# fengweie/UDA_CLR

Measured on AMD Instinct MI355X. Metric: training images/sec (512x512, src+tgt) at 1/2/4/8 MI355X; val Dice vs ref, higher is better.
Workload: dtype f32

## Files before the change

include/uda_clr_hip.h:

```cpp
#ifndef UDA_CLR_HIP_H
#define UDA_CLR_HIP_H

#include <stdint.h>

#ifdef __cplusplus
extern "C" {
#endif

#define UDA_STAT_SLOTS 16

#define UDA_ACT_NONE 0
#define UDA_ACT_RELU 1
#define UDA_ACT_RELU6 2

typedef struct uda_src {
    const float* x;
    int64_t ldx;
    int32_t N, H, W, C;
    const float* scale;
    const float* shift;
    int32_t act;
    int32_t _pad;
    const uint8_t* mask;
    int64_t ldm;
// ... 104 lines not shown
uint64_t uda_conv3n_workspace_bytes(int Cin, int Cout);
int uda_conv3n_wgrad(const uda_src_t* src, const float* dy, int64_t lddy, int Cout, int stride, float* dw,
                     float* workspace, uint64_t workspace_bytes, void* stream);

int uda_relayout_s2d(const float* w, int O, int C, int dgrad, float* out, void* stream);
int uda_s2d_fwd(const float* src, int64_t ld_src, int nchw_in, int N, int Hs, int Ws, int C, int valid_h,
                int valid_w, float slope, float* z, int64_t ld_z, int Hz, int Wz, void* stream);
int uda_s2d_bwd(const float* dz, const float* z_sign, int64_t ld_z, int Hz, int Wz, float slope, int N, int Hs,
                int Ws, int C, int valid_h, int valid_w, float* dst, int64_t ld_dst, int nchw_out, void* stream);
int uda_s2d_bwd_gate(const float* dz, int64_t ld_z, int Hz, int Wz, const float* gate_rows, int64_t ld_gate, float slope,
                     int N, int Hs, int Ws, int C, int valid_h, int valid_w, float* dst, int64_t ld_dst, void* stream);
int uda_x3_pack_s2d_fwd(const float* src, int64_t ld_src, int N, int Hs, int Ws, int C, int valid_h, int valid_w, float slope,
                        int Hz, int Wz, void* out, void* stream);
int uda_x3_pack_s2d_bwd(const float* dz, int64_t ld_z, int Hz, int Wz, const float* gate_rows, int64_t ld_gate, float slope,
                        int N, int Hs, int Ws, int C, int valid_h, int valid_w, void* out, void* stream);

int uda_bn_finalize(const double* stats, int C, double count, const float* gamma, const float* beta,
                    float* running_mean, float* running_var, float momentum, float eps, float* scale,
                    float* shift, float* mean, float* invstd, void* stream);
int uda_bn_running_replay(const float* mean, const float* invstd, int C, double count, int k, float momentum,
                          float eps, float* running_mean, float* running_var, void* stream);
int uda_bn_eval_coeffs(const float* gamma, const float* beta, const float* running_mean,
                       const float* running_var, int C, float eps, float* scale, float* shift,
                       void* stream);
int uda_tn_gain(const double* stats0, const double* stats1, int C, double count0, double count1, float eps,
                float* scale0, float* shift0, float* scale1, float* shift1, float* gain, void* stream);
int uda_tn_eval_coeffs(const float* gamma, const float* beta, const float* running_mean_source,
                       const float* running_var_source, const float* running_mean_target,
                       const float* running_var_target, int C, float eps, float* scale, float* shift, void* stream);
int uda_bn_apply(const uda_src_t* src, const float* residual, int64_t ldr, float* out, int64_t ldo,
// ... 154 lines not shown
```

uda_clr_amd/acts.py:

```python
from __future__ import annotations

from dataclasses import dataclass, field
from typing import Optional

import torch

from .abi import CONSTANTS

ACT_NONE, ACT_RELU, ACT_RELU6 = (CONSTANTS["UDA_ACT_" + a] for a in ("NONE", "RELU", "RELU6"))


def round4(c: int) -> int:
    return (c + 3) // 4 * 4


@dataclass
class BNRec:
    key: str
    mean: torch.Tensor
    invstd: torch.Tensor
    count: float
    q1_border: bool = False
    gain: Optional[torch.Tensor] = None
    frozen: bool = False
# ... 62 lines not shown
    R, T, Cc = w_rtc.shape
    if round4(Cc) < K_CHUNK:
        out = w_rtc.new_zeros(R, T, round4(Cc))
        out[:, :, :Cc] = w_rtc
        return out
    ncc = (Cc + K_CHUNK - 1) // K_CHUNK
    out = w_rtc.new_zeros(R, T, ncc * K_CHUNK)
    out[:, :, :Cc] = w_rtc
    return out.reshape(R, T, ncc, K_CHUNK).permute(0, 2, 1, 3).reshape(R, ncc * T, K_CHUNK).contiguous()


def conv_weight_shape(rows: int, ksize: int, channels: int):
    if ksize == 1 or round4(channels) < K_CHUNK:
        return (rows, ksize * ksize, round4(channels))
    return (rows, ((channels + K_CHUNK - 1) // K_CHUNK) * ksize * ksize, K_CHUNK)
```

uda_clr_amd/csrc/conv_plan.h:

```cpp
#pragma once
#include <stdlib.h>
#include "igemm_args.h"

enum ConvFamily {
    CF_NONE,
    CF_STREAM,
    CF_COUT1,
    CF_HEADS,
    CF_FEW,
    CF_LOW,
    CF_NARROW,
    CF_WS,
    CF_X3,
    CF_X3_TAIL,
    CF_WGRAD,
    CF_WGRAD_WS,
    CF_WGRAD_X3,
    CF_COUNT
};

struct ConvPlan {
    int family;
    const char* error;
    int bm, bn;
// ... 17 lines not shown
    int red_q;
    int stride, Ho, Wo;
    int64_t P;
    int Kc, Jtot;
    size_t lds;
    uint64_t ws_bytes;
};

constexpr size_t igc_tile_bytes(int bm, int bn) { return (size_t)(bm + bn) * IG_LD * sizeof(float); }
constexpr size_t ws_lds_bytes(int bm, int bn) { return 2 * igc_tile_bytes(bm, bn); }
constexpr size_t x3_lds_bytes(int bm, int bn) { return (size_t)2 * (bm + bn) * X3_ROW * 2; }
constexpr size_t wg_ws_lds_bytes(bool big) { return (size_t)2 * WG_BKP * (big ? 512 : 256) * sizeof(float); }
constexpr size_t wg_x3_lds_bytes(int bm, int bn) { return (size_t)2 * 3 * 16 * ((bm * 2 + 64) + (bn * 2 + 64)); }

int launch_conv_ws(ConvKArgs& k, const ConvPlan& p, hipStream_t st);
int launch_conv_x3(const ConvKArgs& k, const ConvPlan& p, const void* x3_src, const void* x3_w, void* ws, hipStream_t st);
int launch_wgrad_ws(WgradKArgs& k, const WgradPlan& p, hipStream_t st);
int launch_wgrad_x3(const WgradKArgs& k, const WgradPlan& p, const void* x3_src, const void* x3_dy, hipStream_t st);

static inline int uda_k_row(int C, int ksize) {
    const int Kc = ((C + 3) / 4) * 4;
    if (ksize == 1 || Kc < IG_BK) return ksize * ksize * Kc;
    return ((Kc + IG_BK - 1) / IG_BK) * ksize * ksize * IG_BK;
}

static bool plan_stream(const uda_conv_args_t* a, int64_t P, int& kh, int& nb) {
    if (a->ksize != 1 || (a->stride > 1) || a->src.mask || a->bias || P < 32768) return false;
    if (!uda_aligned16(a->src.x) || a->src.ldx % 4 || (a->src.C != 16 && a->src.C != 24 && a->src.C != 32)) return false;
    if (P * a->ldy >= ((int64_t)1 << 29) || (a->addend && P * a->ld_add >= ((int64_t)1 << 29))) return false;
    const int C = a->src.C, Cout = a->Cout;
    kh = C / 2;
// ... 218 lines not shown
```

uda_clr_amd/csrc/igemm_args.h:

```cpp
#pragma once
#include "common.h"

struct ConvKArgs {
    uda_src_t src;
    const float* w;
    int Cout, ksize, dil, Kc, Ktot;
    int cen;
    const float* bias;
    const float* addend;
    int64_t ld_add;
    float* y;
    int64_t ldy;
    double* stats;
    int nMt, nNt;
    int debug;
    int x3;
    int stride, Ho, Wo;
};

struct WgradKArgs {
    uda_src_t src;
    const float* dy;
    int64_t lddy;
    int Cout, ksize, dil, Kc, Jtot;
    int cen;
    float* slab;
    int nCot, nJt, chunks_per_split, nchunks;
    int x3;
    int stride, Ho, Wo;
};

#define IG_BK 32
#define IG_LD 36
#define WG_BKP 32
// ... 4 lines not shown
```

uda_clr_amd/csrc/igemm_conv.hip:

```cpp
#include <algorithm>
#include "common.h"
#include "conv_plan.h"

typedef float f32x16 __attribute__((ext_vector_type(16)));


#define IGC_MIN_WAVES(TM, TN, PIPE) ((PIPE) ? 2 : ((TM) * (TN) <= 3 ? 4 : 3))
template <int TM, int TN, int WM, int WN, bool PIPE = false, int XF = -1>
__global__ __launch_bounds__(256) void igemm_conv_kernel(ConvKArgs a) {
    constexpr int BM = 32 * TM * WM, BN = 32 * TN * WN;
    constexpr int A_IT = BM / 32, B_IT = BN / 32;
    constexpr int TILE = (BM + BN) * IG_LD;
    extern __shared__ __attribute__((aligned(16))) float smem[];

    const int tid = threadIdx.x, lane = tid & 63, wave = tid >> 6;
    const int wm = wave / WN, wn = wave % WN;
    const int lid = uda_xcd_remap(blockIdx.x, a.nMt * a.nNt);
    const int mt = lid / a.nNt, nt = lid % a.nNt;
    const int H = a.src.H, W = a.src.W, C = a.src.C;
    const int64_t P = (int64_t)a.src.N * H * W;
    const int64_t m0 = (int64_t)mt * BM;
    const int n0 = nt * BN;

    const int lrow = tid >> 3, kv = (tid & 7) * 4;
// ... 584 lines not shown
        case 122: return launch_stream<12, 2>(k, p.P, st);
        case 123: return launch_stream<12, 3>(k, p.P, st);
        case 125: return launch_stream<12, 5>(k, p.P, st);
        default: return launch_stream<16, 3>(k, p.P, st);
    }
}

extern "C" int uda_conv_uses_x3(const uda_conv_args_t* a) {
    if (!conv_plannable(a)) return 0;
    const int f = conv_plan(a).family;
    return f == CF_X3 || f == CF_X3_TAIL;
}

extern "C" uint64_t uda_conv_fwd_workspace_bytes(const uda_conv_args_t* a) { return conv_plannable(a) ? conv_plan(a).ws_bytes : 0; }

extern "C" int uda_conv_fwd(const uda_conv_args_t* a, void* stream) {
    hipStream_t st = (hipStream_t)stream;
    UDA_REQUIRE(a != nullptr, "uda_conv_fwd: null args");
    if (int e = check_src(a->src, "uda_conv_fwd")) return e;
    UDA_REQUIRE(a->ksize >= 1 && a->ksize <= 3, "uda_conv_fwd: ksize must be 1, 2 or 3");
    UDA_REQUIRE(a->ksize != 2 || a->origin == 0 || a->origin == 1, "uda_conv_fwd: origin must be 0 or 1 for ksize 2");
    UDA_REQUIRE(a->Cout > 0 && a->dil >= 1 && a->y && a->w, "uda_conv_fwd: bad args");
    UDA_REQUIRE(uda_aligned16(a->w), "uda_conv_fwd: weights must be 16-byte aligned");
    UDA_REQUIRE(a->ldy >= a->Cout, "uda_conv_fwd: ldy < Cout");
    UDA_REQUIRE(a->stride <= 2, "uda_conv_fwd: stride must be 1 or 2");
    const int64_t Pin = (int64_t)a->src.N * a->src.H * a->src.W;
    UDA_REQUIRE((Pin + 128) * a->src.ldx < ((int64_t)1 << 29) && (Pin + 128) * (a->src.mask ? a->src.ldm : 1) < ((int64_t)1 << 31),
                "uda_conv_fwd: operand too large for 32-bit byte offsets (P * ld must stay below 2^29 elements)");
    const ConvPlan p = conv_plan(a);
    if (p.error) return uda_set_error("%s", p.error);
    ConvKArgs k;
    k.src = a->src;
    k.stride = p.stride; k.Ho = p.Ho; k.Wo = p.Wo;
    k.w = a->w;
    k.Cout = a->Cout;
    k.ksize = a->ksize;
    k.dil = a->dil;
    k.cen = a->ksize == 3 ? 1 : (a->ksize == 2 ? a->origin : 0);
    k.Kc = p.Kc;
    k.Ktot = p.Ktot;
    k.bias = a->bias;
    k.addend = a->addend;
    k.ld_add = a->ld_add;
    k.y = a->y;
    k.ldy = a->ldy;
// ... 1 lines not shown
    k.debug = 0;
    k.x3 = a->mfma == UDA_MFMA_BF16X3;
    switch (p.family) {
        case CF_STREAM: return launch_stream_shape(k, p, st);
        case CF_COUT1:
            hipLaunchKernelGGL(conv_cout1_kernel, dim3(p.grid), dim3(256), 0, st, k);
            UDA_LAUNCH_CHECK("conv_cout1");
            return 0;
        case CF_HEADS:
            if (p.bn == 1) hipLaunchKernelGGL(conv_heads_kernel<1>, dim3(p.grid), dim3(256), p.lds, st, k);
            else hipLaunchKernelGGL(conv_heads_kernel<2>, dim3(p.grid), dim3(256), p.lds, st, k);
            UDA_LAUNCH_CHECK("conv_heads");
            return 0;
        case CF_FEW: case CF_LOW: case CF_NARROW: return launch_conv_tile(k, p, st);
        case CF_WS: return launch_conv_ws(k, p, st);
        case CF_X3: case CF_X3_TAIL: return launch_conv_x3(k, p, a->x3_src, a->x3_w, a->workspace, st);
        default: return uda_set_error("uda_conv_fwd: no kernel planned");
    }
}



template <int TM, int TN, int WM, int WN>
__global__ __launch_bounds__(256) void igemm_wgrad_kernel(WgradKArgs a) {
    constexpr int BM = 32 * TM * WM, BN = 32 * TN * WN;
    constexpr int AV = BM / 4, BV = BN / 4;
    constexpr int ARPP = 256 / AV, BRPP = 256 / BV;
    constexpr int APASS = WGN_BKP / ARPP, BPASS = WGN_BKP / BRPP;
    __shared__ __attribute__((aligned(16))) float smem[WGN_BKP * (BM + BN)];
    float* As = smem;
    float* Bs = smem + WGN_BKP * BM;

    const int tid = threadIdx.x, lane = tid & 63, wave = tid >> 6;
// ... 366 lines not shown
```

uda_clr_amd/csrc/igemm_x3.hip:

```cpp
#include "common.h"
#include "conv_plan.h"

typedef float f32x16 __attribute__((ext_vector_type(16)));
typedef __bf16 bf16x8 __attribute__((ext_vector_type(8)));
typedef __bf16 bf16x2 __attribute__((ext_vector_type(2)));



__device__ __forceinline__ void x3_split2(float v0, float v1, uint32_t& p1, uint32_t& p2, uint32_t& p3) {
    bf16x2 a = {(__bf16)v0, (__bf16)v1};
    p1 = __builtin_bit_cast(uint32_t, a);
    const float r0 = v0 - __builtin_bit_cast(float, p1 << 16), r1 = v1 - __builtin_bit_cast(float, p1 & 0xffff0000u);
    bf16x2 b = {(__bf16)r0, (__bf16)r1};
    p2 = __builtin_bit_cast(uint32_t, b);
    const float s0 = r0 - __builtin_bit_cast(float, p2 << 16), s1 = r1 - __builtin_bit_cast(float, p2 & 0xffff0000u);
    bf16x2 c = {(__bf16)s0, (__bf16)s1};
    p3 = __builtin_bit_cast(uint32_t, c);
}

struct X3PackArgs {
    uda_src_t src;
    int64_t P;
    int nb;
    uint32_t* out;
// ... 119 lines not shown
    const uint32_t* xa;
    const uint32_t* xw;
    int N, H, W, nbA;
    int stride, Ho, Wo;
    int Cout, ksize, dil, cen, nchunks;
    const float* bias;
    const float* addend;
    int64_t ld_add;
    float* y;
    int64_t ldy;
    double* stats;
    int nMt, nNt;
    int debug;
    int tile_off, ksplit, ntiles_main;
    float* partial;
};

template <int KS, int TN, int BM, bool TAIL = false>
__global__ __launch_bounds__(768) void igemm_conv_x3_kernel(X3KArgs a) {
    constexpr int MW = 8, BN = 64 * TN, TM = 2;
    constexpr int WMM = BM / 64, WNN = MW / WMM, TNW = 2 * TN / WNN;
    static_assert(WMM * WNN == MW && (2 * TN) % WNN == 0, "math-wave grid must tile the workgroup tile");
    constexpr int NTHR = (MW + 4) * 64;
    constexpr int A_U = BM * 6 / 256, B_UNITS = BN * 6, B_U = (B_UNITS + 255) / 256;
    static_assert((BM * 6) % 256 == 0, "A units must divide over the 256 loader threads");
    constexpr bool B_FULL = B_UNITS % 256 == 0;
    constexpr int TILE = (BM + BN) * X3_ROW;
    extern __shared__ __attribute__((aligned(16))) __bf16 smem16[];

    const int tid = threadIdx.x, lane = tid & 63, wave = tid >> 6;
    const bool loader = __builtin_amdgcn_readfirstlane(wave) >= MW;
    const int lid = TAIL ? a.tile_off + (int)blockIdx.x / a.ksplit : uda_xcd_remap(blockIdx.x, a.ntiles_main);
    const int mt = lid / a.nNt, nt = lid % a.nNt;
// ... 163 lines not shown
                a.partial + (int64_t)blockIdx.x * (BM * BN), 0, BM * BN * 4, 0x00020000);
            const int pv = ((wm * 64 + 4 * (lane >> 5)) * BN + wn * (32 * TNW) + (lane & 31)) * 4;
#pragma unroll
            for (int j = 0; j < TNW; ++j)
#pragma unroll
                for (int i = 0; i < TM; ++i)
#pragma unroll
                    for (int r = 0; r < 16; ++r) {
                        const float v = acc[i][j][r];
                        __builtin_amdgcn_raw_buffer_store_b32(__builtin_bit_cast(unsigned, v), pres, pv + 128 * j,
                                                              (32 * i + (r & 3) + 8 * (r >> 2)) * (BN * 4), 0);
                    }
            return;
        }
        if constexpr (TAIL) return;
        float s1[TNW], s2[TNW];
#pragma unroll
        for (int j = 0; j < TNW; ++j) s1[j] = s2[j] = 0.f;
        const int rows_left = (int)min((int64_t)BM, P - m0);
        const int ldy4 = (int)a.ldy * 4, lda4 = (int)a.ld_add * 4;
        const __amdgpu_buffer_rsrc_t yres = __builtin_amdgcn_make_buffer_rsrc(
            a.y + m0 * a.ldy, 0, ((rows_left - 1) * (int)a.ldy + a.Cout) * 4, 0x00020000);
        const __amdgpu_buffer_rsrc_t adres = __builtin_amdgcn_make_buffer_rsrc(
            const_cast<float*>(a.addend ? a.addend + m0 * a.ld_add : a.y), 0, a.addend ? ((rows_left - 1) * (int)a.ld_add + a.Cout) * 4 : 0, 0x00020000);
        const int colb = n0 + wn * (32 * TNW) + (lane & 31);
        const int rbase = wm * 64 + 4 * (lane >> 5);
#pragma unroll
        for (int j = 0; j < TNW; ++j) {
            const int col = colb + 32 * j;
            const bool cok = col < a.Cout;
// ... 40 lines not shown
                atomicAdd(&dst[qd * a.Cout + n0 + cl], (double)t);
            }
        }
    }
}

struct X3TailArgs {
    const float* partial;
    int ksplit, tile_off, ntail, nNt, BM, BN, Cout;
    int64_t P;
    const float* bias;
    const float* addend;
    int64_t ld_add;
    float* y;
    int64_t ldy;
};

__global__ __launch_bounds__(256) void x3_tail_reduce_kernel(X3TailArgs a) {
    const int bn4 = a.BN >> 2, per_tile = a.BM * bn4;
    const int64_t total = (int64_t)a.ntail * per_tile;
    for (int64_t e = (int64_t)blockIdx.x * 256 + threadIdx.x; e < total; e += (int64_t)gridDim.x * 256) {
        const int tl = (int)(e / per_tile), q = (int)(e - (int64_t)tl * per_tile), r = q / bn4, c4 = (q - r * bn4) * 4;
        const int lid = a.tile_off + tl, mt = lid / a.nNt, nt = lid - mt * a.nNt;
        const int64_t row = (int64_t)mt * a.BM + r;
        const int col = nt * a.BN + c4;
        if (row >= a.P || col >= a.Cout) continue;
        float4 acc = make_float4(0.f, 0.f, 0.f, 0.f);
        for (int s = 0; s < a.ksplit; ++s) {
            const float4 v = uda_ld4(a.partial + (((int64_t)tl * a.ksplit + s) * a.BM + r) * a.BN + c4);
            acc.x += v.x; acc.y += v.y; acc.z += v.z; acc.w += v.w;
        }
        const float o[4] = {acc.x, acc.y, acc.z, acc.w};
#pragma unroll
        for (int jj = 0; jj < 4; ++jj)
            if (col + jj < a.Cout) {
                float v = o[jj] + (a.bias ? a.bias[col + jj] : 0.f);
                if (a.addend) v += a.addend[row * a.ld_add + col + jj];
                a.y[row * a.ldy + col + jj] = v;
            }
    }
}

template <int KS, int TN, int BM>
static int launch_x3(X3KArgs& k, const ConvPlan& p, float* ws, hipStream_t st) {
    constexpr int BN = 64 * TN;
    static_assert(x3_lds_bytes(BM, BN) <= 160 * 1024, "tile does not fit the 160 KiB LDS");
    k.nMt = uda_cdiv(p.P, BM);
    k.nNt = uda_cdiv(k.Cout, BN);
    k.debug = 0;
#ifdef UDA_DIAG
    static const int dbg = getenv("UDA_X3_DEBUG") ? atoi(getenv("UDA_X3_DEBUG")) : 0;
    k.debug = dbg;
#endif
    k.tile_off = 0; k.ksplit = 1; k.partial = nullptr;
    k.ntiles_main = p.grid;
    if (k.ntiles_main > 0) {
        if (int e = uda_reserve_lds<igemm_conv_x3_kernel<KS, TN, BM>>(p.lds, "igemm_conv_x3")) return e;
        hipLaunchKernelGGL((igemm_conv_x3_kernel<KS, TN, BM>), dim3(k.ntiles_main), dim3(768), p.lds, st, k);
        UDA_LAUNCH_CHECK("igemm_conv_x3");
    }
    if (p.ksplit > 1) {
        k.tile_off = (int)p.full; k.ksplit = p.ksplit; k.partial = ws;
        if (int e = uda_reserve_lds<igemm_conv_x3_kernel<KS, TN, BM, true>>(p.lds, "igemm_conv_x3 (tail)")) return e;
        hipLaunchKernelGGL((igemm_conv_x3_kernel<KS, TN, BM, true>), dim3((int)p.tail * p.ksplit), dim3(768), p.lds, st, k);
        UDA_LAUNCH_CHECK("igemm_conv_x3 (tail)");
        X3TailArgs r;
        r.partial = k.partial; r.ksplit = p.ksplit; r.tile_off = (int)p.full; r.ntail = (int)p.tail; r.nNt = k.nNt; r.BM = BM; r.BN = BN;
        r.Cout = k.Cout; r.P = p.P; r.bias = k.bias; r.addend = k.addend; r.ld_add = k.ld_add; r.y = k.y; r.ldy = k.ldy;
        const int64_t work = (int64_t)p.tail * BM * (BN / 4);
        hipLaunchKernelGGL(x3_tail_reduce_kernel, dim3((int)uda_cdiv(work, 256)), dim3(256), 0, st, r);
        UDA_LAUNCH_CHECK("x3_tail_reduce");
    }
    return 0;
}

static inline int x3_nb(int C) { return uda_cdiv(C, X3_BK); }

extern "C" uint64_t uda_x3_packed_bytes(int64_t rows, int K) { return (uint64_t)rows * x3_nb(K) * 96 + 64; }

extern "C" int uda_x3_pack(const uda_src_t* src, void* out, void* stream) {
    UDA_REQUIRE(src && src->x && out && uda_aligned16(out) && uda_aligned16(src->x) && src->ldx % 4 == 0 && src->C > 0,
                "uda_x3_pack: bad args (16-byte aligned rows)");
    hipStream_t st = (hipStream_t)stream;
// ... 39 lines not shown
    pa.Hs = Hs; pa.Ws = Ws; pa.Cs = C; pa.vh = valid_h; pa.vw = valid_w; pa.Hz = Hz; pa.Wz = Wz; pa.slope = slope;
    const int64_t tot = pa.P * pa.nb * 2;
    const int grid = (int)(uda_cdiv(tot, 256) > 65536 ? 65536 : uda_cdiv(tot, 256));
    hipLaunchKernelGGL(x3_pack_kernel<4>, dim3(grid), dim3(256), 0, (hipStream_t)stream, pa);
    UDA_LAUNCH_CHECK("x3_pack_s2d_bwd");
    return 0;
}

template <int KS>
static int launch_x3_tile(X3KArgs& x, const ConvPlan& p, float* ws, hipStream_t st) {
    if (p.bn == 64) return launch_x3<3, 1, 256>(x, p, ws, st);
    if (p.bm == 256) return p.bn == 256 ? launch_x3<KS, 4, 256>(x, p, ws, st) : launch_x3<KS, 2, 256>(x, p, ws, st);
    return p.bn == 256 ? launch_x3<KS, 4, 128>(x, p, ws, st) : launch_x3<KS, 2, 128>(x, p, ws, st);
}

int launch_conv_x3(const ConvKArgs& k, const ConvPlan& p, const void* x3_src, const void* x3_w, void* ws, hipStream_t st) {
    const int64_t lim = (int64_t)1 << 31;
    const int nbA = x3_nb(k.src.C), nch = uda_cdiv(k.Ktot, X3_BK);
    UDA_REQUIRE(x3_src && x3_w && uda_aligned16(x3_src) && uda_aligned16(x3_w),
                "uda_conv_fwd (bf16x3): the packed operands x3_src / x3_w are missing (uda_x3_pack; uda_conv_uses_x3 tells when they are needed)");
    const int64_t Pin = (int64_t)k.src.N * k.src.H * k.src.W;
    UDA_REQUIRE((Pin + 256) * nbA * 6 < lim / 16 && (int64_t)(k.Cout + 320) * nch * 6 < lim / 16,
                "uda_conv_fwd (bf16x3): operand too large for the 32-bit offsets of the wide-tile kernel");
    X3KArgs x;
    x.xa = reinterpret_cast<const uint32_t*>(x3_src); x.xw = reinterpret_cast<const uint32_t*>(x3_w);
    x.N = k.src.N; x.H = k.src.H; x.W = k.src.W; x.nbA = nbA;
    x.stride = k.stride; x.Ho = k.Ho; x.Wo = k.Wo;
    x.Cout = k.Cout; x.ksize = k.ksize; x.dil = k.dil; x.cen = k.cen; x.nchunks = nch;
    x.bias = k.bias; x.addend = k.addend; x.ld_add = k.ld_add; x.y = k.y; x.ldy = k.ldy; x.stats = k.stats;
    return p.ks == 3 ? launch_x3_tile<3>(x, p, reinterpret_cast<float*>(ws), st) : launch_x3_tile<1>(x, p, reinterpret_cast<float*>(ws), st);
}

typedef short s16x4 __attribute__((ext_vector_type(4)));
typedef short s16x8 __attribute__((ext_vector_type(8)));

struct X3WgArgs {
    const uint32_t* xdy;
    const uint32_t* xs;
    int N, H, W, nbCo, nbC;
    int stride, Ho, Wo;
    int Cout, Jtot, Kc, ksize, dil, cen;
    float* slab;
    int nCot, nJt, cps, nchunks;
};
// ... 209 lines not shown
```

uda_clr_amd/gan_engine.py:

```python
from __future__ import annotations

import torch

from .acts import Act, round4

SLOPE = 0.2


def _zgrid(v):
    return (v + 5) // 2


class PatchDiscriminatorEngine:
    def __init__(self, kernels):
        self.K = kernels

    def forward(self, x, weights, need_grad, pre_op=0, w_share=None):
        K = self.K
        N, Cc, H, W = x.shape
        src, nchw, Hs, Ws, vh, vw, slope = x, True, H, W, H, W, 1.0
        layers = []
        for li, w in enumerate(weights):
            O = w.shape[0]
            if w_share is None:
# ... 16 lines not shown
            else:
                z = torch.empty((N * Hz * Wz, 4 * Cc), dtype=torch.float32, device=x.device)
                if li == 0 and pre_op:
                    K.adv_s2d_fwd(src, pre_op, z)
                else:
                    K.s2d_fwd(src, nchw, N, Hs, Ws, Cc, vh, vw, slope, z)
            y = torch.empty((N * Hz * Wz, round4(O)), dtype=torch.float32, device=x.device)[:, :O]
            K.conv(Act(z, N, Hz, Wz), wf, 2, 1, y, origin=0)
            keep_gate = need_grad and li > 0 and (packed or getattr(K, "mfma", None) == getattr(K, "MFMA_BF16X3", -1))
            layers.append((z if need_grad else None, Cc, Hs, Ws, vh, vw, Hz, Wz, nchw, wd, src if keep_gate else None))
            src, nchw, Hs, Ws, Cc, slope = y, False, Hz, Wz, O, SLOPE
            vh, vw = vh // 2 + 1, vw // 2 + 1
        out = src.reshape(N, Hs, Ws, Cc)[:, :vh, :vw].permute(0, 3, 1, 2)
        return out, ((layers, N, tuple(x.shape), (x if pre_op else None), pre_op) if need_grad else None)

    def backward(self, ctx, gout, weights, need_x, need_w):
        K = self.K
        layers, N, xshape, x_logits, pre_op = ctx
        z5, C5, Hs5, Ws5, vh5, vw5, Hz, Wz, _, _, _ = layers[-1]
        O = weights[-1].shape[0]
        vh, vw = vh5 // 2 + 1, vw5 // 2 + 1
        dy = torch.zeros((N, Hz, Wz, round4(O)), dtype=torch.float32, device=gout.device)
        dy[:, :vh, :vw, :O] = gout.permute(0, 2, 3, 1)
        dy = dy.reshape(N * Hz * Wz, round4(O))[:, :O]
        dws = [None] * len(weights)
        dx = None
        for l in range(len(weights) - 1, -1, -1):
            z, Cc, Hs, Ws, vh, vw, Hz, Wz, nchw, wd, gate = layers[l]
            w = weights[l]
            O = w.shape[0]
            if need_w:
                dwz = torch.empty((O, 4 * Cc, 2, 2), dtype=torch.float32, device=z.device)
                K.conv_wgrad(Act(z, N, Hz, Wz), dy, 2, 1, dwz, origin=0)
                dws[l] = dwz.reshape(O, 2, 2, Cc, 2, 2).permute(0, 3, 4, 1, 5, 2).reshape(O, Cc, 4, 4)
            if l == 0 and not need_x:
                break
            dz = torch.empty_like(z)
            K.conv(Act(dy, N, Hz, Wz), wd, 2, 1, dz, origin=1)
            if nchw:
                dx = torch.empty(xshape, dtype=torch.float32, device=dz.device)
                if pre_op:
                    K.adv_s2d_bwd(dz, x_logits, pre_op, dx)
                else:
                    K.s2d_bwd(dz, None, 1.0, N, Hs, Ws, Cc, vh, vw, dx, True)
            else:
                below = layers[l - 1]
                need_dx_below = (l - 1 > 0) or need_x
                pack_dy = (gate is not None and hasattr(K, "s2d_pack_bwd") and Cc % 8 == 0
                           and (not need_w or K.wgrad_route_x3(N, Hs, Ws, 4 * below[1], Cc, 2))
                           and (not need_dx_below or K.conv_route_x3(N, Hs, Ws, Cc, 4 * below[1], 2)))
                if pack_dy:
                    dy = K.s2d_pack_bwd(dz, gate, SLOPE, N, Hs, Ws, Cc, vh, vw)
                else:
                    dyn = torch.empty((N * Hs * Ws, round4(Cc)), dtype=torch.float32, device=dz.device)[:, :Cc]
                    if gate is not None:
                        K.s2d_bwd(dz, None, SLOPE, N, Hs, Ws, Cc, vh, vw, dyn, False, gate=gate)
                    else:
                        K.s2d_bwd(dz, z, SLOPE, N, Hs, Ws, Cc, vh, vw, dyn, False)
                    dy = dyn
            del dz
        return dx, (dws if need_w else None)
```

uda_clr_amd/kernels.py:

```python
from __future__ import annotations

import ctypes as C
import math
import os
from typing import Optional

import torch

from .abi import CONSTANTS, STRUCTS, SYMBOLS
from .acts import conv_weight_shape, Act, round4

_LIB_PATH = os.path.join(os.path.dirname(os.path.abspath(__file__)), "lib", "libuda_clr_hip.so")
_lib = None

STAT_SLOTS = CONSTANTS["UDA_STAT_SLOTS"]
FDA_MAX_BAND = CONSTANTS["UDA_FDA_MAX_BAND"]
UdaSrc, UdaConvArgs, UdaWgradArgs = STRUCTS["uda_src_t"], STRUCTS["uda_conv_args_t"], STRUCTS["uda_wgrad_args_t"]


def load_library(path: Optional[str] = None):
    global _lib
    if _lib is not None and path is None:
        return _lib
    path = path or _LIB_PATH
    if not os.path.exists(path):
# ... 195 lines not shown
        if x3_channels:
            lim_rows = min(lim_rows, (self.ELEM_LIMIT // 4) // (((x3_channels + 15) // 16) * 6) - 256)
        if N * rows_per_image <= lim_rows:
            return None
        g = lim_rows // rows_per_image
        if g < 1:
            raise UdaError("one image (%d pixels x %d floats per row) exceeds the 32-bit offsets of the conv kernels" % (rows_per_image, widest_ld))
        return [(n0, min(N, n0 + g)) for n0 in range(0, N, g)]

    @staticmethod
    def _act_rows(a: Act, n0, n1):
        ppi = a.P // a.N
        r = slice(n0 * ppi, n1 * ppi)
        return Act(a.x[r], n1 - n0, a.H, a.W, a.scale, a.shift, a.act, None if a.mask is None else a.mask[r], a.mask_scale, a.bn, a.meta)

    def conv(self, src: Act, w, ksize, dil, out, bias=None, addend=None, stats=None, origin=0, stride=1):
        groups = self._image_groups(src.N, src.P // src.N, max(src.x.stride(0), out.stride(0), 0 if addend is None else addend.stride(0),
                                                               0 if src.mask is None else src.mask.stride(0) // 4),
                                    src.C if self.mfma != self.MFMA_F32 else 0)
        Po = src.N * ((src.H - 1) // stride + 1) * ((src.W - 1) // stride + 1)
        if groups is not None:
            ppo = Po // src.N
            for n0, n1 in groups:
                r = slice(n0 * ppo, n1 * ppo)
                self.conv(self._act_rows(src, n0, n1), w, ksize, dil, out[r], bias, None if addend is None else addend[r], stats, origin, stride)
            return
        a = self._conv_args_of(src, w, ksize, dil, out, bias, addend, stats, origin, stride)
        if self.mfma != self.MFMA_F32 and self.lib.uda_conv_uses_x3(C.byref(a)):
            xs = self._packed(src, a.src, out.device)
            xw = getattr(w, "_x3", None)
            if xw is None:
                xw = self.x3_pack_rows(w)
                w._x3 = xw
            a.x3_src, a.x3_w = xs.data_ptr(), xw.data_ptr()
            nws = int(self.lib.uda_conv_fwd_workspace_bytes(C.byref(a)))
            if nws:
                ws = self._ws(out, nws)
                a.workspace, a.workspace_bytes = ws.data_ptr(), nws
            return self._conv_x3(a)
        self._ck(self.lib.uda_conv_fwd(C.byref(a), self._stream()))

    def conv_args(self, usrc: UdaSrc, Cout, ksize, dil=1, origin=0, stride=1, w=None, bias=None, addend=None, ld_add=0, y=None, ldy=0,
                  stats=None) -> UdaConvArgs:
        a = UdaConvArgs()
        a.src, a.origin = usrc, origin
        a.w, a.Cout, a.ksize, a.dil, a.stride = w, Cout, ksize, dil, stride
        a.bias, a.addend, a.ld_add = bias, addend, ld_add
        a.y, a.ldy, a.stats = y, ldy, stats
        a.mfma = self.mfma
        return a

    def _conv_args_of(self, src: Act, w, ksize, dil, out, bias, addend, stats, origin, stride) -> UdaConvArgs:
        Cout = out.shape[1]
        assert w.is_contiguous() and tuple(w.shape) == conv_weight_shape(Cout, ksize, src.C), \
            "weight layout %s does not match conv %dx%d %d->%d" % (tuple(w.shape), ksize, ksize, src.C, Cout)
        assert out.shape[0] == src.N * ((src.H - 1) // stride + 1) * ((src.W - 1) // stride + 1) and stride in (1, 2)
# ... 8 lines not shown
    def route(self, a) -> str:
        buf = C.create_string_buffer(96)
        if isinstance(a, UdaWgradArgs):
            self.lib.uda_conv_wgrad_route(C.byref(a), buf, len(buf))
        else:
            nws = int(self.lib.uda_conv_fwd_workspace_bytes(C.byref(a)))
            if nws and not a.workspace:
                a.workspace, a.workspace_bytes = 16, nws
            self.lib.uda_conv_route(C.byref(a), buf, len(buf))
        return buf.value.decode()

    def conv_route(self, src: Act, w, ksize, dil, out, bias=None, addend=None, stats=None, origin=0, stride=1) -> str:
        return self.route(self._conv_args_of(src, w, ksize, dil, out, bias, addend, stats, origin, stride))

    def _conv_x3(self, a):
        self._ck(self.lib.uda_conv_fwd(C.byref(a), self._stream()))

    def x3_pack(self, usrc: UdaSrc, rows, K, device):
        out = torch.empty(int(self.lib.uda_x3_packed_bytes(rows, K)), dtype=torch.uint8, device=device)
        self._ck(self.lib.uda_x3_pack(C.byref(usrc), out.data_ptr(), self._stream()))
        return out

    def _packed(self, src: Act, usrc: UdaSrc, device):
        xs = getattr(src, "_x3", None)
        raw = not src.lazy
        if xs is None and raw:
            xs = getattr(src.x, "_x3", None)
        if xs is not None and xs.numel() != int(self.lib.uda_x3_packed_bytes(src.P, src.C)):
            raise RuntimeError("bf16x3 packed operand of %d bytes attached to a [%d, %d] matrix (expected %d): stale attachment"
                               % (xs.numel(), src.P, src.C, int(self.lib.uda_x3_packed_bytes(src.P, src.C))))
# ... 1018 lines not shown
```

Baseline: 376.5.

## Fuse space-to-depth backward and LeakyReLU gating into bf16x3 conv epilogue

```diff
diff --git a/include/uda_clr_hip.h b/include/uda_clr_hip.h
--- a/include/uda_clr_hip.h
+++ b/include/uda_clr_hip.h
@@ -142,6 +142,8 @@
                         int Hz, int Wz, void* out, void* stream);
 int uda_x3_pack_s2d_bwd(const float* dz, int64_t ld_z, int Hz, int Wz, const float* gate_rows, int64_t ld_gate, float slope,
                         int N, int Hs, int Ws, int C, int valid_h, int valid_w, void* out, void* stream);
+int uda_conv_fwd_routed(const uda_conv_args_t* a, const float* gate_rows, int64_t ld_gate, float slope, int Hs, int Ws, int C,
+                        int valid_h, int valid_w, float* dst, int64_t ld_dst, void* dst_packed, void* stream);
 
 int uda_bn_finalize(const double* stats, int C, double count, const float* gamma, const float* beta,
                     float* running_mean, float* running_var, float momentum, float eps, float* scale,
diff --git a/uda_clr_amd/acts.py b/uda_clr_amd/acts.py
--- a/uda_clr_amd/acts.py
+++ b/uda_clr_amd/acts.py
@@ -100,3 +100,10 @@
     if ksize == 1 or round4(channels) < K_CHUNK:
         return (rows, ksize * ksize, round4(channels))
     return (rows, ((channels + K_CHUNK - 1) // K_CHUNK) * ksize * ksize, K_CHUNK)
+
+
+class RoutedOut:
+
+    def __init__(self, gate, slope, N, Hs, Ws, C, vh, vw, dst=None, use_workspace=True):
+        self.gate, self.slope, self.N, self.Hs, self.Ws, self.C, self.vh, self.vw = gate, slope, N, Hs, Ws, C, vh, vw
+        self.dst, self.use_workspace = dst, use_workspace
diff --git a/uda_clr_amd/csrc/conv_plan.h b/uda_clr_amd/csrc/conv_plan.h
--- a/uda_clr_amd/csrc/conv_plan.h
+++ b/uda_clr_amd/csrc/conv_plan.h
@@ -55,7 +55,8 @@
 constexpr size_t wg_x3_lds_bytes(int bm, int bn) { return (size_t)2 * 3 * 16 * ((bm * 2 + 64) + (bn * 2 + 64)); }
 
 int launch_conv_ws(ConvKArgs& k, const ConvPlan& p, hipStream_t st);
-int launch_conv_x3(const ConvKArgs& k, const ConvPlan& p, const void* x3_src, const void* x3_w, void* ws, hipStream_t st);
+int launch_conv_x3(const ConvKArgs& k, const ConvPlan& p, const void* x3_src, const void* x3_w, void* ws, const ConvRouteOut* rt,
+                   hipStream_t st);
 int launch_wgrad_ws(WgradKArgs& k, const WgradPlan& p, hipStream_t st);
 int launch_wgrad_x3(const WgradKArgs& k, const WgradPlan& p, const void* x3_src, const void* x3_dy, hipStream_t st);
 
diff --git a/uda_clr_amd/csrc/igemm_args.h b/uda_clr_amd/csrc/igemm_args.h
--- a/uda_clr_amd/csrc/igemm_args.h
+++ b/uda_clr_amd/csrc/igemm_args.h
@@ -18,6 +18,15 @@
     int stride, Ho, Wo;
 };
 
+struct ConvRouteOut {
+    const float* gate;
+    float* dst;
+    uint32_t* packed;
+    int ldg, ldd, nb;
+    int Hs, Ws, C, vh, vw;
+    float slope;
+};
+
 struct WgradKArgs {
     uda_src_t src;
     const float* dy;
diff --git a/uda_clr_amd/csrc/igemm_conv.hip b/uda_clr_amd/csrc/igemm_conv.hip
--- a/uda_clr_amd/csrc/igemm_conv.hip
+++ b/uda_clr_amd/csrc/igemm_conv.hip
@@ -622,13 +622,12 @@
 
 extern "C" uint64_t uda_conv_fwd_workspace_bytes(const uda_conv_args_t* a) { return conv_plannable(a) ? conv_plan(a).ws_bytes : 0; }
 
-extern "C" int uda_conv_fwd(const uda_conv_args_t* a, void* stream) {
-    hipStream_t st = (hipStream_t)stream;
+static int conv_fwd(const uda_conv_args_t* a, const ConvRouteOut* rt, hipStream_t st) {
     UDA_REQUIRE(a != nullptr, "uda_conv_fwd: null args");
     if (int e = check_src(a->src, "uda_conv_fwd")) return e;
     UDA_REQUIRE(a->ksize >= 1 && a->ksize <= 3, "uda_conv_fwd: ksize must be 1, 2 or 3");
     UDA_REQUIRE(a->ksize != 2 || a->origin == 0 || a->origin == 1, "uda_conv_fwd: origin must be 0 or 1 for ksize 2");
-    UDA_REQUIRE(a->Cout > 0 && a->dil >= 1 && a->y && a->w, "uda_conv_fwd: bad args");
+    UDA_REQUIRE(a->Cout > 0 && a->dil >= 1 && (a->y || rt) && a->w, "uda_conv_fwd: bad args");
     UDA_REQUIRE(uda_aligned16(a->w), "uda_conv_fwd: weights must be 16-byte aligned");
     UDA_REQUIRE(a->ldy >= a->Cout, "uda_conv_fwd: ldy < Cout");
     UDA_REQUIRE(a->stride <= 2, "uda_conv_fwd: stride must be 1 or 2");
@@ -637,6 +636,15 @@
                 "uda_conv_fwd: operand too large for 32-bit byte offsets (P * ld must stay below 2^29 elements)");
     const ConvPlan p = conv_plan(a);
     if (p.error) return uda_set_error("%s", p.error);
+    if (rt) {
+        UDA_REQUIRE(p.family == CF_X3 || p.family == CF_X3_TAIL,
+                    "uda_conv_fwd_routed: these arguments do not run on the bf16x3 wide-tile kernel (uda_conv_uses_x3)");
+        UDA_REQUIRE(rt->Hs <= 2 * p.Ho - 2 && rt->Ws <= 2 * p.Wo - 2,
+                    "uda_conv_fwd_routed: source rows beyond 2*Hz - 3 or columns beyond 2*Wz - 3 are reached by no z element and would stay undefined");
+        const int64_t reach = (int64_t)a->src.N * rt->Hs * rt->Ws + 4 * rt->Ws;
+        UDA_REQUIRE(reach * rt->ldg < ((int64_t)1 << 29) && reach * (rt->packed ? (int64_t)rt->nb * 24 : (int64_t)rt->ldd) < ((int64_t)1 << 29),
+                    "uda_conv_fwd_routed: destination too large for 32-bit byte offsets");
+    }
     ConvKArgs k;
     k.src = a->src;
     k.stride = p.stride; k.Ho = p.Ho; k.Wo = p.Wo;
@@ -668,9 +676,33 @@
             return 0;
         case CF_FEW: case CF_LOW: case CF_NARROW: return launch_conv_tile(k, p, st);
         case CF_WS: return launch_conv_ws(k, p, st);
-        case CF_X3: case CF_X3_TAIL: return launch_conv_x3(k, p, a->x3_src, a->x3_w, a->workspace, st);
+        case CF_X3: case CF_X3_TAIL: return launch_conv_x3(k, p, a->x3_src, a->x3_w, a->workspace, rt, st);
         default: return uda_set_error("uda_conv_fwd: no kernel planned");
     }
+}
+
+extern "C" int uda_conv_fwd(const uda_conv_args_t* a, void* stream) { return conv_fwd(a, nullptr, (hipStream_t)stream); }
+
+extern "C" int uda_conv_fwd_routed(const uda_conv_args_t* a, const float* gate_rows, int64_t ld_gate, float slope, int Hs, int Ws, int C,
+                                   int valid_h, int valid_w, float* dst, int64_t ld_dst, void* dst_packed, void* stream) {
+    UDA_REQUIRE(a != nullptr, "uda_conv_fwd_routed: null args");
+    UDA_REQUIRE(a->ksize == 2 && a->origin == 1 && a->stride <= 1, "uda_conv_fwd_routed: needs ksize 2, origin 1, stride 1 (an input gradient on the z grid)");
+    UDA_REQUIRE(!a->stats && !a->bias && !a->addend, "uda_conv_fwd_routed: stats, bias and addend cannot be combined with a routed output");
+    UDA_REQUIRE(C > 0 && C % 32 == 0 && a->Cout == 4 * C,
+                "uda_conv_fwd_routed: needs Cout == 4*C and C %% 32 == 0 (a 32-column block lies inside one (a, b) group, whole 16-wide packed blocks)");
+    UDA_REQUIRE((dst != nullptr) != (dst_packed != nullptr), "uda_conv_fwd_routed: exactly one of dst and dst_packed");
+    UDA_REQUIRE(gate_rows && uda_aligned16(gate_rows) && ld_gate >= C && ld_gate % 4 == 0,
+                "uda_conv_fwd_routed: gate_rows must be 16-byte aligned rows of at least C floats");
+    UDA_REQUIRE(dst ? (uda_aligned16(dst) && ld_dst >= C && ld_dst % 4 == 0) : uda_aligned16(dst_packed),
+                "uda_conv_fwd_routed: dst must be 16-byte aligned (rows of at least C floats)");
+    UDA_REQUIRE(a->src.N > 0 && Hs > 0 && Ws > 0 && valid_h > 0 && valid_w > 0 && valid_h <= Hs && valid_w <= Ws &&
+                a->src.H == (valid_h + 5) / 2 && a->src.W == (valid_w + 5) / 2,
+                "uda_conv_fwd_routed: bad geometry (src must live on the z grid of the valid region)");
+    ConvRouteOut rt;
+    rt.gate = gate_rows; rt.dst = dst; rt.ldg = (int)ld_gate; rt.ldd = (int)ld_dst;
+    rt.packed = reinterpret_cast<uint32_t*>(dst_packed); rt.nb = C / X3_BK;
+    rt.Hs = Hs; rt.Ws = Ws; rt.C = C; rt.vh = valid_h; rt.vw = valid_w; rt.slope = slope;
+    return conv_fwd(a, &rt, (hipStream_t)stream);
 }
 
 
diff --git a/uda_clr_amd/csrc/igemm_x3.hip b/uda_clr_amd/csrc/igemm_x3.hip
--- a/uda_clr_amd/csrc/igemm_x3.hip
+++ b/uda_clr_amd/csrc/igemm_x3.hip
@@ -4,6 +4,7 @@
 typedef float f32x16 __attribute__((ext_vector_type(16)));
 typedef __bf16 bf16x8 __attribute__((ext_vector_type(8)));
 typedef __bf16 bf16x2 __attribute__((ext_vector_type(2)));
+typedef unsigned u32x4 __attribute__((ext_vector_type(4)));
 
 
 
@@ -157,9 +158,19 @@
     int debug;
     int tile_off, ksplit, ntiles_main;
     float* partial;
+    ConvRouteOut rt;
 };
 
-template <int KS, int TN, int BM, bool TAIL = false>
+__device__ __forceinline__ void x3_route_row(int64_t p, int64_t P, int Hz, int Wz, int Hs, int Ws, int& pix, int& h0, int& w0) {
+    pix = 0; h0 = w0 = -(1 << 20);
+    if (p < P) {
+        const int q = (int)p, j = q % Wz, t = q / Wz, i = t % Hz, n = t / Hz;
+        h0 = 2 * i - 2; w0 = 2 * j - 2;
+        pix = (n * Hs + h0) * Ws + w0;
+    }
+}
+
+template <int KS, int TN, int BM, bool TAIL = false, int RT = 0>
 __global__ __launch_bounds__(768) void igemm_conv_x3_kernel(X3KArgs a) {
     constexpr int MW = 8, BN = 64 * TN, TM = 2;
     constexpr int WMM = BM / 64, WNN = MW / WMM, TNW = 2 * TN / WNN;
@@ -353,6 +364,115 @@
             return;
         }
         if constexpr (TAIL) return;
+        if constexpr (RT != 0) {
+            const ConvRouteOut& rt = a.rt;
+            const int wv = __builtin_amdgcn_readfirstlane(wave);
+            int2* tab = reinterpret_cast<int2*>(smem16) + wv * 64;
+            const int dpix = RT == 2 ? rt.nb * 96 : rt.ldd * 4, gpix = rt.ldg * 4;
+            {
+                int pix, h0, w0;
+                x3_route_row(m0 + wm * 64 + lane, P, a.Ho, a.Wo, rt.Hs, rt.Ws, pix, h0, w0);
+                int inb = 0, okb = 0;
+#pragma unroll
+                for (int ab = 0; ab < 4; ++ab) {
+                    const int h = h0 + (ab >> 1), w = w0 + (ab & 1);
+                    const bool in = h >= 0 && h < rt.Hs && w >= 0 && w < rt.Ws;
+                    inb |= (in ? 1 : 0) << ab;
+                    okb |= (in && h < rt.vh && w < rt.vw ? 1 : 0) << ab;
+                }
+                tab[lane] = make_int2(pix * dpix | inb, pix * gpix | okb);
+            }
+            const int64_t npix = (int64_t)a.N * rt.Hs * rt.Ws;
+            const __amdgpu_buffer_rsrc_t dres = RT == 2
+                ? __builtin_amdgcn_make_buffer_rsrc(rt.packed, 0, (int)(npix * dpix), 0x00020000)
+                : __builtin_amdgcn_make_buffer_rsrc(rt.dst, 0, (int)(((npix - 1) * rt.ldd + rt.C) * 4), 0x00020000);
+            const __amdgpu_buffer_rsrc_t gres = __builtin_amdgcn_make_buffer_rsrc(
+                const_cast<float*>(rt.gate), 0, (int)(((npix - 1) * rt.ldg + rt.C) * 4), 0x00020000);
+            const int2* trow = tab + 4 * (lane >> 5);
+            uint32_t* stage = reinterpret_cast<uint32_t*>(smem16) + MW * 64 * 2 + wv * (32 * 48);
+            static_assert(RT != 2 || MW * 64 * 8 + MW * 32 * 192 <= 2 * TILE * 2, "row table and stage must fit the tile images");
+            constexpr int NU = TNW * TM * 2;
+            constexpr bool PARK = RT == 2 && BM == 256 && TN == 4;
+            float* park = reinterpret_cast<float*>(smem16) + MW * 64 * 2 + MW * 32 * 48 + wv * 64 + lane;
+            static_assert(!PARK || MW * 64 * 8 + MW * 32 * 192 + 16 * MW * 64 * 4 <= 2 * TILE * 2, "parked block must fit the tile images");
+            if constexpr (PARK) {
+#pragma unroll
+                for (int r = 0; r < 16; ++r) park[r * (MW * 64)] = acc[TM - 1][TNW - 1][r];
+            }
+            int inbit = 0, okbit = 0, dcol = 0, gcol = 0;
+            auto columns = [&](int u) {
+                const int col0 = __builtin_amdgcn_readfirstlane(n0 + wn * (32 * TNW) + 32 * (u / (2 * TM)));
+                const int ab = (col0 >= rt.C) + (col0 >= 2 * rt.C) + (col0 >= 3 * rt.C) + (col0 >= 4 * rt.C);
+                const int c0 = col0 - ab * rt.C, pixo = (ab >> 1) * rt.Ws + (ab & 1);
+                inbit = okbit = ab < 4 ? 1 << ab : 0;
+                gcol = pixo * gpix + (c0 + (lane & 31)) * 4;
+                dcol = RT == 2 ? pixo * dpix + (c0 >> 4) * 96 : pixo * dpix + (c0 + (lane & 31)) * 4;
+            };
+            auto rl_of = [](int u, int k) { const int r = 8 * (u & 1) + k; return 32 * ((u >> 1) % TM) + (r & 3) + 8 * (r >> 2); };
+            auto issue = [&](int u, float (&g)[8]) {
+                columns(u);
+#pragma unroll
+                for (int k = 0; k < 8; ++k) {
+                    const int2 t = trow[rl_of(u, k)];
+                    g[k] = __builtin_bit_cast(float, __builtin_amdgcn_raw_buffer_load_b32(gres, (t.y & okbit) ? (t.y & ~15) + gcol : OOB, 0, 0));
+                }
+            };
+            auto value = [&](int u, int k, float g, const int2& t) {
+                const int i = (u >> 1) % TM, j = u / (2 * TM), r = 8 * (u & 1) + k;
+                float v = (PARK && i == TM - 1 && j == TNW - 1 ? park[r * (MW * 64)] : acc[i][j][r]) + 0.f;
+                if (!(g > 0.f)) v *= rt.slope;
+                return (t.y & okbit) ? v : 0.f;
+            };
+            auto finish = [&](int u, const float (&g)[8]) {
+                columns(u);
+                if constexpr (RT == 1) {
+#pragma unroll
+                    for (int k = 0; k < 8; ++k) {
+                        const int2 t = trow[rl_of(u, k)];
+                        const float v = value(u, k, g[k], t);
+                        __builtin_amdgcn_raw_buffer_store_b32(__builtin_bit_cast(unsigned, v), dres, (t.x & inbit) ? (t.x & ~15) + dcol : OOB, 0, 0);
+                    }
+                } else {
+                    const bool even = !(lane & 1);
+#pragma unroll
+                    for (int k = 0; k < 8; k += 2) {
+                        if (BM == 256 && k) asm volatile("" ::: "memory");
+                        const int rlA = rl_of(u, k), rlB = rl_of(u, k + 1);
+                        const float vA = value(u, k, g[k], trow[rlA]), vB = value(u, k + 1, g[k + 1], trow[rlB]);
+                        const float mine = even ? vA : vB, other = __shfl_xor(even ? vB : vA, 1);
+                        uint32_t p1, p2, p3;
+                        x3_split2(even ? mine : other, even ? other : mine, p1, p2, p3);
+                        const int rb = ((even ? rlA : rlB) & 31) + 4 * (lane >> 5);
+                        uint32_t* d = stage + rb * 48 + ((lane & 31) >> 4) * 24 + ((lane & 15) >> 1);
+                        d[0] = p1; d[8] = p2; d[16] = p3;
+                    }
+                    if (u & 1) {
+                        const int rband = 32 * ((u >> 1) % TM);
+#pragma unroll
+                        for (int k = 0; k < 6; ++k) {
+                            if (k == 2 || k == 4) asm volatile("" ::: "memory");
+                            const int e = lane + 64 * k, run = e / 12, part = e - run * 12;
+                            const int2 t = tab[rband + run];
+                            const u32x4 v = *reinterpret_cast<const u32x4*>(stage + 4 * e);
+                            __builtin_amdgcn_raw_buffer_store_b128(v, dres, (t.x & inbit) ? (t.x & ~15) + dcol + part * 16 : OOB, 0, 0);
+                        }
+                    }
+                }
+            };
+            constexpr int D = (BM == 256 && TN == 4) ? 2 : 4;
+            float g[D][8];
+#pragma unroll
+            for (int u = 0; u < D - 1; ++u)
+                if (u < NU) issue(u, g[u]);
+#pragma unroll
+            for (int u = 0; u < NU; ++u) {
+                asm volatile("" ::: "memory");
+                if (u + D - 1 < NU) issue(u + D - 1, g[(u + D - 1) % D]);
+                asm volatile("" ::: "memory");
+                finish(u, g[u % D]);
+            }
+            return;
+        }
         float s1[TNW], s2[TNW];
 #pragma unroll
         for (int j = 0; j < TNW; ++j) s1[j] = s2[j] = 0.f;
@@ -423,6 +543,8 @@
     int64_t ld_add;
     float* y;
     int64_t ldy;
+    int routed, Hz, Wz;
+    ConvRouteOut rt;
 };
 
 __global__ __launch_bounds__(256) void x3_tail_reduce_kernel(X3TailArgs a) {
@@ -440,6 +562,34 @@
             acc.x += v.x; acc.y += v.y; acc.z += v.z; acc.w += v.w;
         }
         const float o[4] = {acc.x, acc.y, acc.z, acc.w};
+        if (a.routed) {
+            int pix, h0, w0;
+            x3_route_row(row, a.P, a.Hz, a.Wz, a.rt.Hs, a.rt.Ws, pix, h0, w0);
+            const int ab = col / a.rt.C, c = col - ab * a.rt.C, h = h0 + (ab >> 1), w = w0 + (ab & 1);
+            if (h < 0 || h >= a.rt.Hs || w < 0 || w >= a.rt.Ws) continue;
+            const int64_t px = pix + (ab >> 1) * a.rt.Ws + (ab & 1);
+            float4 v = make_float4(0.f, 0.f, 0.f, 0.f);
+            if (h < a.rt.vh && w < a.rt.vw) {
+                const float4 g = uda_ld4(a.rt.gate + px * a.rt.ldg + c);
+                v = make_float4(o[0] + 0.f, o[1] + 0.f, o[2] + 0.f, o[3] + 0.f);
+                if (!(g.x > 0.f)) v.x *= a.rt.slope;
+                if (!(g.y > 0.f)) v.y *= a.rt.slope;
+                if (!(g.z > 0.f)) v.z *= a.rt.slope;
+                if (!(g.w > 0.f)) v.w *= a.rt.slope;
+            }
+            if (a.rt.packed) {
+                uint32_t p1[2], p2[2], p3[2];
+                x3_split2(v.x, v.y, p1[0], p2[0], p3[0]);
+                x3_split2(v.z, v.w, p1[1], p2[1], p3[1]);
+                uint32_t* d = a.rt.packed + ((px * a.rt.nb + (c >> 4)) * 24 + ((c & 15) >> 1));
+                *reinterpret_cast<uint2*>(d) = make_uint2(p1[0], p1[1]);
+                *reinterpret_cast<uint2*>(d + 8) = make_uint2(p2[0], p2[1]);
+                *reinterpret_cast<uint2*>(d + 16) = make_uint2(p3[0], p3[1]);
+            } else {
+                uda_st4(a.rt.dst + px * a.rt.ldd + c, v);
+            }
+            continue;
+        }
 #pragma unroll
         for (int jj = 0; jj < 4; ++jj)
             if (col + jj < a.Cout) {
@@ -450,7 +600,7 @@
     }
 }
 
-template <int KS, int TN, int BM>
+template <int KS, int TN, int BM, int RT = 0>
 static int launch_x3(X3KArgs& k, const ConvPlan& p, float* ws, hipStream_t st) {
     constexpr int BN = 64 * TN;
     static_assert(x3_lds_bytes(BM, BN) <= 160 * 1024, "tile does not fit the 160 KiB LDS");
@@ -464,8 +614,8 @@
     k.tile_off = 0; k.ksplit = 1; k.partial = nullptr;
     k.ntiles_main = p.grid;
     if (k.ntiles_main > 0) {
-        if (int e = uda_reserve_lds<igemm_conv_x3_kernel<KS, TN, BM>>(p.lds, "igemm_conv_x3")) return e;
-        hipLaunchKernelGGL((igemm_conv_x3_kernel<KS, TN, BM>), dim3(k.ntiles_main), dim3(768), p.lds, st, k);
+        if (int e = uda_reserve_lds<igemm_conv_x3_kernel<KS, TN, BM, false, RT>>(p.lds, "igemm_conv_x3")) return e;
+        hipLaunchKernelGGL((igemm_conv_x3_kernel<KS, TN, BM, false, RT>), dim3(k.ntiles_main), dim3(768), p.lds, st, k);
         UDA_LAUNCH_CHECK("igemm_conv_x3");
     }
     if (p.ksplit > 1) {
@@ -476,6 +626,7 @@
         X3TailArgs r;
         r.partial = k.partial; r.ksplit = p.ksplit; r.tile_off = (int)p.full; r.ntail = (int)p.tail; r.nNt = k.nNt; r.BM = BM; r.BN = BN;
         r.Cout = k.Cout; r.P = p.P; r.bias = k.bias; r.addend = k.addend; r.ld_add = k.ld_add; r.y = k.y; r.ldy = k.ldy;
+        r.routed = RT != 0; r.Hz = k.Ho; r.Wz = k.Wo; r.rt = k.rt;
         const int64_t work = (int64_t)p.tail * BM * (BN / 4);
         hipLaunchKernelGGL(x3_tail_reduce_kernel, dim3((int)uda_cdiv(work, 256)), dim3(256), 0, st, r);
         UDA_LAUNCH_CHECK("x3_tail_reduce");
@@ -545,7 +696,14 @@
     return p.bn == 256 ? launch_x3<KS, 4, 128>(x, p, ws, st) : launch_x3<KS, 2, 128>(x, p, ws, st);
 }
 
-int launch_conv_x3(const ConvKArgs& k, const ConvPlan& p, const void* x3_src, const void* x3_w, void* ws, hipStream_t st) {
+template <int RT>
+static int launch_x3_routed(X3KArgs& x, const ConvPlan& p, float* ws, hipStream_t st) {
+    if (p.bm == 256) return p.bn == 256 ? launch_x3<3, 4, 256, RT>(x, p, ws, st) : launch_x3<3, 2, 256, RT>(x, p, ws, st);
+    return p.bn == 256 ? launch_x3<3, 4, 128, RT>(x, p, ws, st) : launch_x3<3, 2, 128, RT>(x, p, ws, st);
+}
+
+int launch_conv_x3(const ConvKArgs& k, const ConvPlan& p, const void* x3_src, const void* x3_w, void* ws, const ConvRouteOut* rt,
+                   hipStream_t st) {
     const int64_t lim = (int64_t)1 << 31;
     const int nbA = x3_nb(k.src.C), nch = uda_cdiv(k.Ktot, X3_BK);
     UDA_REQUIRE(x3_src && x3_w && uda_aligned16(x3_src) && uda_aligned16(x3_w),
@@ -559,6 +717,11 @@
     x.stride = k.stride; x.Ho = k.Ho; x.Wo = k.Wo;
     x.Cout = k.Cout; x.ksize = k.ksize; x.dil = k.dil; x.cen = k.cen; x.nchunks = nch;
     x.bias = k.bias; x.addend = k.addend; x.ld_add = k.ld_add; x.y = k.y; x.ldy = k.ldy; x.stats = k.stats;
+    x.rt = rt ? *rt : ConvRouteOut{};
+    if (rt) {
+        UDA_REQUIRE(p.ks == 3 && p.bn >= 128, "uda_conv_fwd_routed: no routed epilogue for this tile");
+        return rt->packed ? launch_x3_routed<2>(x, p, reinterpret_cast<float*>(ws), st) : launch_x3_routed<1>(x, p, reinterpret_cast<float*>(ws), st);
+    }
     return p.ks == 3 ? launch_x3_tile<3>(x, p, reinterpret_cast<float*>(ws), st) : launch_x3_tile<1>(x, p, reinterpret_cast<float*>(ws), st);
 }
 
diff --git a/uda_clr_amd/gan_engine.py b/uda_clr_amd/gan_engine.py
--- a/uda_clr_amd/gan_engine.py
+++ b/uda_clr_amd/gan_engine.py
@@ -2,7 +2,7 @@
 
 import torch
 
-from .acts import Act, round4
+from .acts import Act, RoutedOut, round4
 
 SLOPE = 0.2
 
@@ -54,7 +54,7 @@
         out = src.reshape(N, Hs, Ws, Cc)[:, :vh, :vw].permute(0, 3, 1, 2)
         return out, ((layers, N, tuple(x.shape), (x if pre_op else None), pre_op) if need_grad else None)
 
-    def backward(self, ctx, gout, weights, need_x, need_w):
+    def backward(self, ctx, gout, weights, need_x, need_w, fuse_route=True):
         K = self.K
         layers, N, xshape, x_logits, pre_op = ctx
         z5, C5, Hs5, Ws5, vh5, vw5, Hz, Wz, _, _, _ = layers[-1]
@@ -75,6 +75,17 @@
                 dws[l] = dwz.reshape(O, 2, 2, Cc, 2, 2).permute(0, 3, 4, 1, 5, 2).reshape(O, Cc, 4, 4)
             if l == 0 and not need_x:
                 break
+            below = None if nchw else layers[l - 1]
+            pack_dy = (not nchw and gate is not None and hasattr(K, "s2d_pack_bwd") and Cc % 8 == 0
+                       and (not need_w or K.wgrad_route_x3(N, Hs, Ws, 4 * below[1], Cc, 2))
+                       and (not ((l - 1 > 0) or need_x) or K.conv_route_x3(N, Hs, Ws, Cc, 4 * below[1], 2)))
+            if (fuse_route and not nchw and gate is not None and Cc % 32 == 0 and hasattr(K, "conv_routed")
+                    and (pack_dy or l == 1) and K.conv_route_x3(N, Hz, Wz, O, 4 * Cc, 2)):
+                dst = None if pack_dy else torch.empty((N * Hs * Ws, round4(Cc)), dtype=torch.float32, device=gout.device)[:, :Cc]
+                shape = torch.empty((N * Hz * Wz, 4 * Cc), dtype=torch.float32, device="meta")
+                res = K.conv(Act(dy, N, Hz, Wz), wd, 2, 1, shape, origin=1, routed=RoutedOut(gate, SLOPE, N, Hs, Ws, Cc, vh, vw, dst))
+                dy = res if pack_dy else dst
+                continue
             dz = torch.empty_like(z)
             K.conv(Act(dy, N, Hz, Wz), wd, 2, 1, dz, origin=1)
             if nchw:
@@ -84,11 +95,6 @@
                 else:
                     K.s2d_bwd(dz, None, 1.0, N, Hs, Ws, Cc, vh, vw, dx, True)
             else:
-                below = layers[l - 1]
-                need_dx_below = (l - 1 > 0) or need_x
-                pack_dy = (gate is not None and hasattr(K, "s2d_pack_bwd") and Cc % 8 == 0
-                           and (not need_w or K.wgrad_route_x3(N, Hs, Ws, 4 * below[1], Cc, 2))
-                           and (not need_dx_below or K.conv_route_x3(N, Hs, Ws, Cc, 4 * below[1], 2)))
                 if pack_dy:
                     dy = K.s2d_pack_bwd(dz, gate, SLOPE, N, Hs, Ws, Cc, vh, vw)
                 else:
diff --git a/uda_clr_amd/kernels.py b/uda_clr_amd/kernels.py
--- a/uda_clr_amd/kernels.py
+++ b/uda_clr_amd/kernels.py
@@ -8,7 +8,7 @@
 import torch
 
 from .abi import CONSTANTS, STRUCTS, SYMBOLS
-from .acts import conv_weight_shape, Act, round4
+from .acts import conv_weight_shape, Act, RoutedOut, round4
 
 _LIB_PATH = os.path.join(os.path.dirname(os.path.abspath(__file__)), "lib", "libuda_clr_hip.so")
 _lib = None
@@ -234,7 +234,9 @@
         r = slice(n0 * ppi, n1 * ppi)
         return Act(a.x[r], n1 - n0, a.H, a.W, a.scale, a.shift, a.act, None if a.mask is None else a.mask[r], a.mask_scale, a.bn, a.meta)
 
-    def conv(self, src: Act, w, ksize, dil, out, bias=None, addend=None, stats=None, origin=0, stride=1):
+    def conv(self, src: Act, w, ksize, dil, out, bias=None, addend=None, stats=None, origin=0, stride=1, routed=None):
+        if routed is not None:
+            return self.conv_routed(src, w, out, routed)
         groups = self._image_groups(src.N, src.P // src.N, max(src.x.stride(0), out.stride(0), 0 if addend is None else addend.stride(0),
                                                                0 if src.mask is None else src.mask.stride(0) // 4),
                                     src.C if self.mfma != self.MFMA_F32 else 0)
@@ -260,6 +262,37 @@
             return self._conv_x3(a)
         self._ck(self.lib.uda_conv_fwd(C.byref(a), self._stream()))
 
+    def conv_routed(self, src: Act, w, out, routed: "RoutedOut"):
+        r = routed
+        Hz, Wz = (r.vh + 5) // 2, (r.vw + 5) // 2
+        assert (src.N, src.H, src.W) == (r.N, Hz, Wz) and tuple(out.shape) == (src.P, 4 * r.C) and r.gate.shape == (r.N * r.Hs * r.Ws, r.C)
+        assert not src.lazy and tuple(w.shape) == conv_weight_shape(4 * r.C, 2, src.C) and w.is_contiguous()
+        dev = src.x.device
+        a = self.conv_args(self._src(src), 4 * r.C, 2, 1, 1, 1, w.data_ptr(), None, None, 0, None, out.stride(0), None)
+        if not self.lib.uda_conv_uses_x3(C.byref(a)):
+            raise UdaError("conv_routed: a conv of %d -> %d channels on %d pixels does not run on the bf16x3 wide-tile kernel" % (src.C, 4 * r.C, src.P))
+        xs = self._packed(src, a.src, dev)
+        xw = getattr(w, "_x3", None)
+        if xw is None:
+            xw = self.x3_pack_rows(w)
+            w._x3 = xw
+        a.x3_src, a.x3_w = xs.data_ptr(), xw.data_ptr()
+        nws = int(self.lib.uda_conv_fwd_workspace_bytes(C.byref(a)))
+        if nws and r.use_workspace:
+            ws = self._ws(src.x, nws)
+            a.workspace, a.workspace_bytes = ws.data_ptr(), nws
+        gp, ldg = _mat(r.gate, "gate")
+        res = None
+        if r.dst is None:
+            res, xd = self._packed_only(r.N * r.Hs * r.Ws, r.C, dev)
+            dst = (None, 0, xd.data_ptr())
+        else:
+            assert r.dst.shape == r.gate.shape
+            dst = _mat(r.dst, "dst") + (None,)
+        a._routed = (gp, ldg, float(r.slope), r.Hs, r.Ws, r.C, r.vh, r.vw) + dst
+        self._conv_x3(a)
+        return res
+
     def conv_args(self, usrc: UdaSrc, Cout, ksize, dil=1, origin=0, stride=1, w=None, bias=None, addend=None, ld_add=0, y=None, ldy=0,
                   stats=None) -> UdaConvArgs:
         a = UdaConvArgs()
@@ -298,6 +331,9 @@
         return self.route(self._conv_args_of(src, w, ksize, dil, out, bias, addend, stats, origin, stride))
 
     def _conv_x3(self, a):
+        routed = getattr(a, "_routed", None)
+        if routed is not None:
+            return self._ck(self.lib.uda_conv_fwd_routed(C.byref(a), *routed, self._stream()))
         self._ck(self.lib.uda_conv_fwd(C.byref(a), self._stream()))
 
     def x3_pack(self, usrc: UdaSrc, rows, K, device):
```

After: 380.7, median of 6. 1.01x the previous value.
